# AndyWu0719/Audio-CALM

Measured on NVIDIA B200. Metric: log-mel audio-hours/sec, higher is better.
Workload: dtype f32

## Files before the change

### audio-calm_b200/csrc/acb_kernels.cu

```cuda
#include "audiocalm_b200.h"
#include "acb_fft32.cuh"

#include <cuda_bf16.h>
#include <cuda_runtime.h>

#include <algorithm>
#include <cmath>
#include <cstdio>
#include <cstring>
#include <mutex>
#include <numeric>
#include <string>
#include <vector>

namespace acb {

constexpr int kNfft = 1024;
constexpr int kHop = 256;
constexpr int kBins = 512;
constexpr int kTileFrames = 8;
constexpr int kGroupWarps = 4;
constexpr int kGroupThreads = kGroupWarps * 32;
constexpr int kMaxGroups = 4;
constexpr int kTileSamples = (kTileFrames + 3) * kHop;
constexpr int kRowStride = 36;
constexpr int kPlaneFloats = 32 * kRowStride;
constexpr int kScratchFloats = 2 * kPlaneFloats + 8;
constexpr int kSlots = 8;
constexpr int kMaxMels = 128;
constexpr int kMaxRounds = 4;
constexpr int kMaxWeights = 4096;
constexpr int kOutStageOffset = 2 * kBins;
static_assert(kScratchFloats % 32 == 8 && kScratchFloats % 4 == 0, "pair stride must be 8 (mod 32) words and 16-byte aligned");
static_assert(kOutStageOffset + kTileFrames * (kMaxMels | 1) <= kScratchFloats, "staged tile must fit above the power spectrum");

thread_local std::string g_last_error;

int fail(int code, const std::string& msg) {
    g_last_error = msg;
    return code;
}
static int cuda_fail(cudaError_t e, const char* what) {
    g_last_error = std::string(what) + ": " + cudaGetErrorString(e);
    return ACB_ERR_CUDA;
}
#define ACB_CUDA(call)                                  \
    do {                                                \
        cudaError_t e__ = (call);                       \
        if (e__ != cudaSuccess) return cuda_fail(e__, #call); \
    } while (0)

__device__ __forceinline__ unsigned smem_addr(const void* p) { return static_cast<unsigned>(__cvta_generic_to_shared(p)); }
__device__ __forceinline__ void mbar_init(unsigned long long* bar, unsigned count) {
    asm volatile("mbarrier.init.shared::cta.b64 [%0], %1;" ::"r"(smem_addr(bar)), "r"(count) : "memory");
}
__device__ __forceinline__ void mbar_arrive(unsigned long long* bar) {
    asm volatile("mbarrier.arrive.shared::cta.b64 _, [%0];" ::"r"(smem_addr(bar)) : "memory");
}
__device__ __forceinline__ void mbar_arrive_expect_tx(unsigned long long* bar, unsigned bytes) {
    asm volatile("mbarrier.arrive.expect_tx.shared::cta.b64 _, [%0], %1;" ::"r"(smem_addr(bar)), "r"(bytes) : "memory");
}
__device__ __forceinline__ bool mbar_wait(unsigned long long* bar, unsigned parity) {
    unsigned ok = 0;
    for (int spin = 0; spin < (1 << 26) && !ok; ++spin) {
        asm volatile("{\n\t.reg .pred p;\n\tmbarrier.try_wait.parity.shared::cta.b64 p, [%1], %2;\n\tselp.u32 %0, 1, 0, p;\n\t}\n"
                     : "=r"(ok) : "r"(smem_addr(bar)), "r"(parity) : "memory");
    }
    return ok != 0;
}
__device__ __forceinline__ void bulk_copy_g2s(void* smem, const void* gmem, unsigned bytes, unsigned long long* bar) {
    asm volatile("cp.async.bulk.shared::cluster.global.mbarrier::complete_tx::bytes [%0], [%1], %2, [%3];"
                 ::"r"(smem_addr(smem)), "l"(gmem), "r"(bytes), "r"(smem_addr(bar)) : "memory");
}

struct LogmelParams {
    const float* window;
    const float4* twiddle;
    const float* plan_w;
    const int* plan_woff;
    const short* plan_trip;
    const short* plan_band;
    const short* plan_astart;
    int n_plan_w;
    int n_mels;
    float clamp_min;
    float log_scale;
    float log_floor;
    const float* wav;
    const long long* clip_offset;
    const long long* clip_length;
    long long clip_stride;
    long long uniform_length;
    const int* tile_start;
    int n_clips;
    int n_tiles;
    int uniform_tiles_per_clip;
    const float* clip_peak;
    void* out;
    int out_bf16;
    int time_major;
    const long long* out_offset;
    long long out_clip_stride;
    long long frame_capacity;
    const long long* frame_capacity_per_clip;
    int pad_multiple;
    int fill_tail;
    float fill_value;
    int affine;
    float affine_mean;
    float affine_inv_std;
    const float* bin_mean;
    const float* bin_std;
    double* moments_partial;
    int* error_flag;
};

struct SmemLayout {
    int samples, scratch, twiddle, window, plan_w, affine, plan_rec, mbar, moments, total_bytes;
};

__host__ __device__ inline int out_row_stride(int n_mels) { return n_mels | 1; }

__host__ __device__ inline SmemLayout make_smem_layout(int kGroups, int n_mels, int n_plan_w, bool with_moments = false) {
    SmemLayout L;
    int off = 0;
    L.samples = off; off += kGroups * kTileSamples;
    L.scratch = off; off += kGroups * kGroupWarps * kScratchFloats;
    L.twiddle = off; off += 5 * 32 * 4;
    L.window = off; off += 32 * 20;
    if (!with_moments) {
        L.plan_rec = off; off += kGroupWarps * kMaxRounds * kSlots * 4;
        L.mbar = off; off += 2 * kGroups;
        off = (off + 3) & ~3;
        L.affine = off; off += 2 * kMaxMels;
        L.plan_w = off; off += (n_plan_w + 3) & ~3;
        L.moments = off;
    } else {
        L.plan_w = off; off += (n_plan_w + 3) & ~3;
        L.affine = off; off += 2 * ((n_mels + 1) & ~1);
        off = (off + 3) & ~3;
        L.plan_rec = off; off += kGroupWarps * kMaxRounds * kSlots * 4;
        L.mbar = off; off += 2 * kGroups;
        L.moments = off; off += kGroups * 4 * n_mels;
    }
    L.total_bytes = off * 4;
    return L;
}

struct ClipCursor {
    long long wav_base;
    long long length;
    long long out_base;
    int cap;
    int frames;
    int frames_padded;
    int clip;
    int tile_in_clip;
    int tiles_in_clip;
    float gain;
};

__device__ __forceinline__ void cursor_load_clip(const LogmelParams& p, ClipCursor& c) {
    const int i = c.clip;
    c.wav_base = p.clip_offset ? p.clip_offset[i] : (long long)i * p.clip_stride;
    c.length = p.clip_length ? p.clip_length[i] : p.uniform_length;
    c.out_base = p.out_offset ? p.out_offset[i] : (long long)i * p.out_clip_stride;
    c.cap = (int)(p.frame_capacity_per_clip ? p.frame_capacity_per_clip[i] : p.frame_capacity);
    c.frames = 1 + (int)(c.length / kHop);
    const int rem = c.frames % p.pad_multiple;
    c.frames_padded = rem ? c.frames + (p.pad_multiple - rem) : c.frames;
    c.tiles_in_clip = p.tile_start ? (__ldg(p.tile_start + i + 1) - __ldg(p.tile_start + i)) : p.uniform_tiles_per_clip;
    c.gain = 1.f;
    if (p.clip_peak) {
        const float peak = __ldg(p.clip_peak + i);
        if (peak > 0.f) {
            const float s = 0.95f / (peak + 1e-8f);
            c.gain = s * s;
        }
    }
}

__device__ __forceinline__ void cursor_init(const LogmelParams& p, ClipCursor& c, long long tile) {
    if (p.tile_start == nullptr) {
        c.clip = (int)(tile / p.uniform_tiles_per_clip);
        c.tile_in_clip = (int)(tile - (long long)c.clip * p.uniform_tiles_per_clip);
    } else {
        int lo = 0, hi = p.n_clips;
        while (hi - lo > 1) {
            const int mid = (lo + hi) >> 1;
            if ((long long)__ldg(p.tile_start + mid) <= tile) lo = mid; else hi = mid;
        }
        c.clip = lo;
        c.tile_in_clip = (int)(tile - __ldg(p.tile_start + lo));
    }
    cursor_load_clip(p, c);
}

__device__ __forceinline__ void cursor_advance(const LogmelParams& p, ClipCursor& c) {
    if (++c.tile_in_clip >= c.tiles_in_clip) {
        c.tile_in_clip = 0;
        do { ++c.clip; cursor_load_clip(p, c); } while (c.tiles_in_clip == 0 && c.clip + 1 < p.n_clips);
    }
}

__device__ __forceinline__ void group_sync(int grp) {
    asm volatile("bar.sync %0, %1;" ::"r"(grp + 1), "n"(kGroupThreads) : "memory");
}

__device__ __noinline__ void gather_edge_tile(const float* __restrict__ src, long long g0, long long L, float* s_samples, int gt) {
    static_assert(kTileSamples % kGroupThreads == 0, "whole rounds");
    float v[kTileSamples / kGroupThreads];
#pragma unroll
    for (int k = 0; k < kTileSamples / kGroupThreads; ++k) {
        long long idx = g0 + gt + k * kGroupThreads;
        if (idx < 0) idx = -idx;
        if (idx >= L) idx = 2 * (L - 1) - idx;
        v[k] = (idx >= 0 && idx < L) ? __ldg(src + idx) : 0.f;
    }
#pragma unroll
    for (int k = 0; k < kTileSamples / kGroupThreads; ++k) s_samples[gt + k * kGroupThreads] = v[k];
}

__device__ __forceinline__ void load_tile_samples(const LogmelParams& p, const ClipCursor& t, float* s_samples, int gt, int grp,
                                                  unsigned long long* full) {
    const int f0 = t.tile_in_clip * kTileFrames;
    const long long g0 = (long long)f0 * kHop - kNfft / 2;
    const float* src = p.wav + t.wav_base;
// ... 65 lines not shown
            v = p.fill_value;
        } else {
            continue;
        }
        const size_t e0 = p.time_major ? ((size_t)fr * n_mels + b) : ((size_t)b * c.cap + fr);
        out[e0] = to_out<OutT>(v);
        if (dup) {
            const int fd = 2 * T - 2 - fr;
            const size_t e1 = p.time_major ? ((size_t)fd * n_mels + b) : ((size_t)b * c.cap + fd);
            out[e1] = to_out<OutT>(v);
        }
    }
}

template <typename OutT>
__device__ __forceinline__ void fill_span(OutT* ptr, long long n, OutT fv, int t, int nt) {
    constexpr int per16 = 16 / (int)sizeof(OutT);
    const long long head = min(n, (long long)(((16 - (reinterpret_cast<uintptr_t>(ptr) & 15)) & 15) / sizeof(OutT)));
    for (long long i = t; i < head; i += nt) ptr[i] = fv;
    const long long body = (n - head) / per16;
    unsigned w;
    if (sizeof(OutT) == 4) w = *reinterpret_cast<const unsigned*>(&fv);
    else { const unsigned short h = *reinterpret_cast<const unsigned short*>(&fv); w = (unsigned)h | ((unsigned)h << 16); }
    uint4* q = reinterpret_cast<uint4*>(ptr + head);
    for (long long i = t; i < body; i += nt) q[i] = make_uint4(w, w, w, w);
    for (long long i = head + body * per16 + t; i < n; i += nt) ptr[i] = fv;
}

template <typename OutT>
__device__ __forceinline__ void fill_row_tail(const LogmelParams& p, const ClipCursor& c, int n_mels, int tid) {
    const int f_begin = (c.tile_in_clip + 1) * kTileFrames;
    const long long n_fill = (long long)c.cap - f_begin;
    if (n_fill <= 0) return;
    OutT* out = reinterpret_cast<OutT*>(p.out) + c.out_base;
    const OutT fv = to_out<OutT>(p.fill_value);
    if (p.time_major) {
        fill_span<OutT>(out + (size_t)f_begin * n_mels, n_fill * n_mels, fv, tid, kGroupThreads);
    } else {
        const int lane = tid & 31, warp = tid >> 5;
        for (int b = warp; b < n_mels; b += kGroupWarps) fill_span<OutT>(out + (size_t)b * c.cap + f_begin, n_fill, fv, lane, 32);
    }
}

__device__ __forceinline__ float lg2_normal(float x) {
    float y;
    asm("lg2.approx.ftz.f32 %0, %1;" : "=f"(y) : "f"(x));
    return y;
}

__device__ __forceinline__ void two_sum_add(float2& acc, float x) {
    const float t = __fadd_rn(acc.x, x);
    const float bb = __fsub_rn(t, acc.x);
    const float e = __fadd_rn(__fsub_rn(acc.x, __fsub_rn(t, bb)), __fsub_rn(x, bb));
    acc.y = __fadd_rn(acc.y, e);
    acc.x = t;
}

template <int G, bool kMoments, typename OutT>
__global__ void __launch_bounds__(G * kGroupThreads, G == 4 ? 1 : 2) logmel_fused_kernel(const LogmelParams p) {
    constexpr int kGroups = G;
    constexpr int kThreads = G * kGroupThreads;
    extern __shared__ __align__(16) float smem[];
    const SmemLayout L = make_smem_layout(G, p.n_mels, p.n_plan_w, kMoments);
    const int tid = threadIdx.x;
    const int lane = tid & 31;
    const int grp = tid / kGroupThreads;
    const int gt = tid % kGroupThreads;
    const int gw = gt >> 5;
    const int n_mels = p.n_mels;
    const int S = out_row_stride(n_mels);
    const bool write_out = p.out != nullptr;

    float* s_samples = smem + L.samples + grp * kTileSamples;
    float* s_scratch = smem + L.scratch + grp * kGroupWarps * kScratchFloats;
    float* s_out = s_scratch + kOutStageOffset;
    float4* s_tw4 = reinterpret_cast<float4*>(smem + L.twiddle);
    float* s_win = smem + L.window;
    float* s_pw = smem + L.plan_w;
    float2* s_aff = reinterpret_cast<float2*>(smem + L.affine);
    int4* s_rec = reinterpret_cast<int4*>(smem + L.plan_rec);
    float2* s_mom = reinterpret_cast<float2*>(smem + L.moments) + grp * 2 * n_mels;
    unsigned long long* s_full = reinterpret_cast<unsigned long long*>(smem + L.mbar) + grp;

    for (int i = tid; i < 5 * 32; i += kThreads) s_tw4[i] = p.twiddle[i];
    for (int i = tid; i < kNfft / 2; i += kThreads)
        s_win[(i & 31) * 20 + (i >> 5)] = p.window[i];
    for (int i = tid; i < p.n_plan_w; i += kThreads) s_pw[i] = p.plan_w[i];
    for (int i = tid; i < kGroupWarps * kMaxRounds * kSlots; i += kThreads) {
        const int slot = i / kSlots, qq = i - slot * kSlots;
        s_rec[i] = make_int4(p.plan_astart[i] >> 1, (p.plan_woff[slot] >> 1) + qq, p.plan_band[i], p.plan_trip[slot]);
    }
    for (int i = tid; i < n_mels; i += kThreads) {
        float sc = 1.f, sh = 0.f;
        if (p.affine == 1) { sc = p.affine_inv_std; sh = -p.affine_mean * p.affine_inv_std; }
        else if (p.affine == 2) { sc = 1.f / __ldg(p.bin_std + i); sh = -__ldg(p.bin_mean + i) * sc; }
        s_aff[i] = make_float2(sc, sh);
    }
    if (kMoments)
        for (int i = gt; i < 2 * n_mels; i += kGroupThreads) s_mom[i] = make_float2(0.f, 0.f);
    if (gt == 0) {
        mbar_init(s_full, 1);
        asm volatile("fence.mbarrier_init.release.cluster;" ::: "memory");
    }
    __syncthreads();

    const long long n_groups = (long long)gridDim.x * kGroups, g_index = (long long)blockIdx.x * kGroups + grp;
    const long long t_begin = (long long)p.n_tiles * g_index / n_groups;
    const long long t_end = (long long)p.n_tiles * (g_index + 1) / n_groups;

    ClipCursor cur;
    bool staged = false;
    unsigned full_parity = 0;
    if (t_begin < t_end) {
        cursor_init(p, cur, t_begin);
        staged = cur.tile_in_clip * kTileFrames < cur.frames;
        if (staged) load_tile_samples(p, cur, s_samples, gt, grp, s_full);
    }

    const int q = lane >> 2;
    const int pl = lane & 3;
    const float* pair_scratch = s_scratch + pl * kScratchFloats;
    float* scr = s_scratch + gw * kScratchFloats;
    float2* scr2 = reinterpret_cast<float2*>(scr);

    for (long long tile = t_begin; tile < t_end; ++tile) {
        if (staged) {
            if (!mbar_wait(s_full, full_parity) && lane == 0) atomicExch(p.error_flag, 1);
            full_parity ^= 1;
        }

        const int f0 = cur.tile_in_clip * kTileFrames;
        const bool has_frames = f0 < cur.frames;
        const bool active = has_frames && f0 + 2 * gw < cur.frames;

        if (active) {
            float2 pr[16], pi[16];
            {
                const float* sp = s_samples + (2 * gw) * kHop + lane;
                float2 v[20];
#pragma unroll
                for (int r = 0; r < 20; ++r) v[r] = make_float2(sp[32 * (2 * r)], sp[32 * (2 * r + 1)]);
                float4 w4[4];
                const float4* wq = reinterpret_cast<const float4*>(s_win + lane * 20);
#pragma unroll
                for (int u = 0; u < 4; ++u) w4[u] = wq[u];
#pragma unroll
                for (int j = 0; j < 8; ++j) {
                    const int t = brev5(2 * j) >> 1;
                    const float2 wa = (t & 1) ? make_float2(w4[t >> 1].z, w4[t >> 1].w) : make_float2(w4[t >> 1].x, w4[t >> 1].y);
                    const float2 br = __ffma2_rn(neg2(v[t + 8]), wa, v[t + 8]), bi = __ffma2_rn(neg2(v[t + 12]), wa, v[t + 12]);
                    pr[2 * j] = __ffma2_rn(v[t], wa, br);
                    pr[2 * j + 1] = __ffma2_rn(v[t], wa, neg2(br));
                    pi[2 * j] = __ffma2_rn(v[t + 4], wa, bi);
                    pi[2 * j + 1] = __ffma2_rn(v[t + 4], wa, neg2(bi));
                }
            }
            fft32_packed_from_stage2(pr, pi);
            group_sync(grp);
            {
                float* pre = scr + lane;
                float* pim = scr + kPlaneFloats + lane;
                float2 tr[4], ti[4];
#pragma unroll
                for (int c = 0; c < 4; ++c) {
                    const float4 sd = s_tw4[c * 32 + lane];
                    tr[c] = make_float2(sd.x, sd.y);
                    ti[c] = make_float2(sd.z, sd.w);
                }
                const float4 w4 = s_tw4[4 * 32 + lane];
                const float2 w4r = bcast2(w4.x), w4i = bcast2(w4.y);
#pragma unroll
                for (int k = 0; k < 16; ++k) {
                    const int c = k & 3;
                    const float2 yr = __ffma2_rn(neg2(pi[k]), ti[c], __fmul2_rn(pr[k], tr[c]));
                    const float2 yi = __ffma2_rn(pr[k], ti[c], __fmul2_rn(pi[k], tr[c]));
                    pre[k * kRowStride] = yr.x;
                    pre[(k + 16) * kRowStride] = yr.y;
                    pim[k * kRowStride] = yi.x;
                    pim[(k + 16) * kRowStride] = yi.y;
                    if (k + 4 < 16) {
                        const float2 nr = __ffma2_rn(neg2(ti[c]), w4i, __fmul2_rn(tr[c], w4r));
                        ti[c] = __ffma2_rn(tr[c], w4i, __fmul2_rn(ti[c], w4r));
                        tr[c] = nr;
                    }
                }
            }
            __syncwarp();
            {
                const float4* re4 = reinterpret_cast<const float4*>(scr + lane * kRowStride);
                const float4* im4 = reinterpret_cast<const float4*>(scr + kPlaneFloats + lane * kRowStride);
#pragma unroll
                for (int h = 0; h < 8; ++h) {
                    const float4 zr = re4[h], zi = im4[h];
                    pr[brev3(h)] = make_float2(zr.x, zr.y);
                    pr[brev3(h) + 8] = make_float2(zr.z, zr.w);
                    pi[brev3(h)] = make_float2(zi.x, zi.y);
                    pi[brev3(h) + 8] = make_float2(zi.z, zi.w);
                }
            }
// ... 454 lines not shown
                    T v[4];
#pragma unroll
                    for (int j = 0; j < 4; ++j) { const long long f = s0 + t + j; v[j] = (f >= 0 && f < n) ? src[f] : padv; }
                    *reinterpret_cast<float4*>(dst + t) = make_float4(v[0], v[1], v[2], v[3]);
                }
            }
        } else {
            for (long long t = lane; t < out_frames; t += 32) {
                const long long f = s0 + t;
                dst[t] = (f >= 0 && f < n) ? src[f] : padv;
            }
        }
    }
}

template <typename T>
__global__ void __launch_bounds__(256) pad_transpose_kernel(const T* __restrict__ feat, const long long* __restrict__ row_offset,
                                                            const long long* __restrict__ lens, int dim, T* __restrict__ out,
                                                            long long out_frames, float pad_value,
                                                            const long long* __restrict__ mask_start, const long long* __restrict__ mask_len) {
    constexpr int kT = 64;
    __shared__ float tile[kT][kT + 1];
    const int clip = blockIdx.z;
    const long long t0 = (long long)blockIdx.x * kT;
    const int d0 = blockIdx.y * kT;
    const long long n = lens[clip];
    const T* src = feat + row_offset[clip] * dim;
    const long long m0 = mask_start ? mask_start[clip] : 0, m1 = mask_start ? m0 + mask_len[clip] : 0;
    const int q = threadIdx.x & 15, r0 = threadIdx.x >> 4;
    const bool vec_in = sizeof(T) == 4 && (dim & 3) == 0 && (reinterpret_cast<uintptr_t>(src) & 15) == 0;
#pragma unroll
    for (int pass = 0; pass < kT / 16; ++pass) {
        const int r = pass * 16 + r0;
        const long long t = t0 + r;
        const int d = d0 + 4 * q;
        float v[4] = {pad_value, pad_value, pad_value, pad_value};
        if (t < n) {
            const bool masked = t >= m0 && t < m1;
            if (vec_in && d + 3 < dim) {
                if constexpr (sizeof(T) == 4) {
                    const float4 u = __ldg(reinterpret_cast<const float4*>(src + t * dim + d));
                    v[0] = u.x; v[1] = u.y; v[2] = u.z; v[3] = u.w;
                }
            } else {
#pragma unroll
                for (int j = 0; j < 4; ++j) if (d + j < dim) v[j] = (float)src[t * dim + d + j];
            }
            if (masked) { v[0] = v[1] = v[2] = v[3] = 0.f; }
        }
#pragma unroll
        for (int j = 0; j < 4; ++j) tile[4 * q + j][r] = v[j];
    }
    __syncthreads();
    const bool vec_out = sizeof(T) == 4 && (out_frames & 3) == 0 && (reinterpret_cast<uintptr_t>(out) & 15) == 0;
#pragma unroll
    for (int pass = 0; pass < kT / 16; ++pass) {
        const int r = pass * 16 + r0;
        const int d = d0 + r;
        const long long t = t0 + 4 * q;
        if (d >= dim || t >= out_frames) continue;
        T* dst = out + ((long long)clip * dim + d) * out_frames + t;
        if (vec_out && t + 3 < out_frames) {
            if constexpr (sizeof(T) == 4)
                *reinterpret_cast<float4*>(dst) = make_float4(tile[r][4 * q], tile[r][4 * q + 1], tile[r][4 * q + 2], tile[r][4 * q + 3]);
        } else {
#pragma unroll
            for (int j = 0; j < 4; ++j) if (t + j < out_frames) dst[j] = from_float<T>(tile[r][4 * q + j]);
        }
    }
}

}

struct acb_frontend {
    int device = 0;
    int n_fft = 0, hop = 0, n_mels = 0, n_weights = 0, log_kind = 0;
    float clamp_min = 0.f;
    int num_sms = 0;
    int groups = 0;
    int grid = 0;
    int smem_bytes = 0;
    int smem_bytes_moments = 0;
    void* d_blob = nullptr;
    const float* d_window = nullptr;
    const float4* d_twiddle = nullptr;
    const float* d_plan_w = nullptr;
    const int* d_plan_woff = nullptr;
    const short* d_plan_trip = nullptr;
    const short* d_plan_band = nullptr;
    const short* d_plan_astart = nullptr;
    int n_plan_w = 0;
    int* d_err = nullptr;
    cudaStream_t s_in = nullptr, s_out = nullptr;
    std::vector<cudaEvent_t> ev;
    std::mutex mu;
};

using namespace acb;

extern "C" {

int acb_abi_version(void) { return ACB_ABI_VERSION; }
const char* acb_last_error(void) { return g_last_error.c_str(); }
int acb_frames_per_tile(void) { return kTileFrames; }

int64_t acb_frames_for_length(int64_t length, int n_fft, int hop) {
    if (n_fft <= 0 || hop <= 0) return -1;
    if (length <= n_fft / 2) return -1;
    return 1 + length / hop;
}

int64_t acb_padded_frames(int64_t frames, int multiple) {
    if (multiple <= 1) return frames;
    const int64_t r = frames % multiple;
    return r ? frames + (multiple - r) : frames;
}

int64_t acb_plan_tiles(const int64_t* lengths_host, int32_t n_clips, int n_fft, int hop, int64_t frame_capacity,
                       int32_t* tile_start_host) {
    if (!lengths_host || !tile_start_host || n_clips < 0) return fail(ACB_ERR_INVALID, "acb_plan_tiles: null argument");
    int64_t total = 0;
    for (int32_t i = 0; i < n_clips; ++i) {
        const int64_t T = acb_frames_for_length(lengths_host[i], n_fft, hop);
        if (T < 0) {
            return fail(ACB_ERR_INVALID, "acb_plan_tiles: clip " + std::to_string(i) + " has " + std::to_string(lengths_host[i]) +
                                             " samples; reflect padding needs more than " + std::to_string(n_fft / 2));
        }
        const int64_t cover = frame_capacity > 0 ? frame_capacity : T;
        tile_start_host[i] = (int32_t)total;
        total += (cover + kTileFrames - 1) / kTileFrames;
        if (total > INT32_MAX) return fail(ACB_ERR_INVALID, "acb_plan_tiles: more than 2^31 tiles in one call");
    }
    tile_start_host[n_clips] = (int32_t)total;
    return total;
}

int acb_frontend_create(acb_frontend** out, int device, int n_fft, int hop, int n_mels, const float* window_host,
                        const float* fb_host, float clamp_min, int log_kind) {
    if (!out || !window_host || !fb_host) return fail(ACB_ERR_INVALID, "acb_frontend_create: null argument");
    if (n_fft != kNfft || hop != kHop)
        return fail(ACB_ERR_UNSUPPORTED, "acb_frontend_create: this build has kernels for n_fft=1024, hop=256 only (got n_fft=" +
                                             std::to_string(n_fft) + ", hop=" + std::to_string(hop) + ")");
    if (n_mels < 1 || n_mels > kMaxMels) return fail(ACB_ERR_UNSUPPORTED, "acb_frontend_create: n_mels must be in [1, 128]");
    if (log_kind != ACB_LOG_NATURAL && log_kind != ACB_LOG_10) return fail(ACB_ERR_INVALID, "acb_frontend_create: bad log_kind");
    if (!(clamp_min >= 1.17549435e-38f)) return fail(ACB_ERR_INVALID, "acb_frontend_create: clamp_min must be a positive normal float");
    for (int n = 0; n < kNfft / 2; ++n) {
        const double dev = std::fabs((double)window_host[n + kNfft / 2] - (1.0 - (double)window_host[n]));
        if (!(dev <= 1e-6))
            return fail(ACB_ERR_UNSUPPORTED, "acb_frontend_create: the window must have the periodic-Hann property w[n + 512] = 1 - w[n] "
                                             "(deviation " + std::to_string(dev) + " at n=" + std::to_string(n) + ")");
    }
    const int n_freq = n_fft / 2 + 1;

    std::vector<int> start(n_mels, 0), len(n_mels, 0), off(n_mels, 0);
    std::vector<float> weights;
    for (int m = 0; m < n_mels; ++m) {
        int lo = -1, hi = -1;
        for (int f = 0; f < n_freq; ++f)
            if (fb_host[(size_t)f * n_mels + m] != 0.f) { if (lo < 0) lo = f; hi = f; }
        off[m] = (int)weights.size();
        if (lo >= 0) {
            if (hi >= kBins) {
                if (fb_host[(size_t)(n_freq - 1) * n_mels + m] != 0.f)
                    return fail(ACB_ERR_UNSUPPORTED, "acb_frontend_create: filterbank has weight on the Nyquist bin");
            }
            start[m] = lo;
            len[m] = hi - lo + 1;
            for (int f = lo; f <= hi; ++f) weights.push_back(fb_host[(size_t)f * n_mels + m] * 0.25f);
        }
    }
    if ((int)weights.size() > kMaxWeights) return fail(ACB_ERR_UNSUPPORTED, "acb_frontend_create: filterbank too dense");

    std::vector<int> alen(n_mels), aend(n_mels);
// ... 2 lines not shown
        aend[m] = (start[m] + std::max(len[m], 1) + 1) & ~1;
        alen[m] = aend[m] - (start[m] & ~1);
    }
    std::vector<int> order(n_mels);
    std::iota(order.begin(), order.end(), 0);
    std::stable_sort(order.begin(), order.end(), [&](int a, int b) { return alen[a] > alen[b]; });
    const int n_rounds = (n_mels + kSlots - 1) / kSlots;
    std::vector<short> plan_band(kGroupWarps * kMaxRounds * kSlots, (short)-1), plan_astart(kGroupWarps * kMaxRounds * kSlots, (short)0),
        plan_trip(kGroupWarps * kMaxRounds, (short)0);
    std::vector<int> plan_woff(kGroupWarps * kMaxRounds, 0);
    std::vector<float> plan_w;
    std::vector<int> load(kGroupWarps, 0), rounds(kGroupWarps, 0);
    for (int g = 0; g < n_rounds; ++g) {
        int best = -1;
        for (int w = 0; w < kGroupWarps; ++w)
            if (rounds[w] < kMaxRounds && (best < 0 || load[w] < load[best])) best = w;
        if (best < 0) return fail(ACB_ERR_UNSUPPORTED, "acb_frontend_create: mel plan overflow");
        std::vector<int> par[2];
        for (int q = 0; q < kSlots && kSlots * g + q < n_mels; ++q) {
            const int m = order[kSlots * g + q];
            par[((start[m] & ~1) >> 1) & 1].push_back(m);
        }
        std::vector<int> slots;
        while (!par[0].empty() && !par[1].empty()) {
            slots.push_back(par[0].back()); par[0].pop_back();
            slots.push_back(par[1].back()); par[1].pop_back();
        }
        for (int k = 0; k < 2; ++k)
            for (int m : par[k]) slots.push_back(m);
        std::vector<int> shift(slots.size(), 0), as(slots.size(), 0);
        int trip = 2;
        for (int iter = 0; iter < 8; ++iter) {
            trip = 2;
            for (size_t i = 0; i < slots.size(); ++i) trip = std::max(trip, aend[slots[i]] - ((start[slots[i]] & ~1) - shift[i]));
            for (size_t i = 0; i < slots.size(); ++i) {
                as[i] = (start[slots[i]] & ~1) - shift[i];
                if (as[i] + trip > kBins) as[i] = std::max(0, (kBins - trip) & ~1);
            }
            bool changed = false;
            for (size_t i = 0; i + 1 < slots.size(); i += 2) {
                if ((((as[i] >> 1) ^ (as[i + 1] >> 1)) & 1) != 0) continue;
                const size_t x = (as[i + 1] >= 2 && (start[slots[i + 1]] & ~1) - shift[i + 1] == as[i + 1]) ? i + 1
                                 : ((as[i] >= 2 && (start[slots[i]] & ~1) - shift[i] == as[i]) ? i : slots.size());
                if (x < slots.size()) { shift[x] += 2; changed = true; }
            }
            if (!changed) break;
        }
        const int slot = best * kMaxRounds + rounds[best];
        plan_trip[slot] = (short)trip;
        plan_woff[slot] = (int)plan_w.size();
        plan_w.resize(plan_w.size() + (size_t)trip * kSlots, 0.f);
        float* wbase = plan_w.data() + plan_woff[slot];
        for (size_t q = 0; q < slots.size(); ++q) {
            const int m = slots[q];
            plan_band[slot * kSlots + q] = (short)m;
            plan_astart[slot * kSlots + q] = (short)as[q];
            for (int i = 0; i < len[m]; ++i) {
                const int rel = start[m] + i - as[q];
                if (rel < 0 || rel >= trip) return fail(ACB_ERR_UNSUPPORTED, "acb_frontend_create: mel plan window error");
                wbase[(rel >> 1) * (2 * kSlots) + q * 2 + (rel & 1)] = weights[off[m] + i];
            }
        }
        load[best] += trip + 16;
        rounds[best]++;
    }
    if ((int)plan_w.size() > kMaxWeights * 4) return fail(ACB_ERR_UNSUPPORTED, "acb_frontend_create: mel plan too large");

    std::vector<float4> tw(5 * 32);
    for (int l = 0; l < 32; ++l) {
        auto wre = [&](int m) { return (float)cos(-2.0 * M_PI * (double)(m * l) / 1024.0); };
        auto wim = [&](int m) { return (float)sin(-2.0 * M_PI * (double)(m * l) / 1024.0); };
        for (int k = 0; k < 4; ++k) tw[k * 32 + l] = make_float4(wre(k), wre(k + 16), wim(k), wim(k + 16));
        tw[4 * 32 + l] = make_float4(wre(4), wim(4), 0.f, 0.f);
    }

    int prev = 0;
    ACB_CUDA(cudaGetDevice(&prev));
    ACB_CUDA(cudaSetDevice(device));
    auto* fe = new acb_frontend();
    fe->device = device; fe->n_fft = n_fft; fe->hop = hop; fe->n_mels = n_mels; fe->n_weights = (int)weights.size();
    fe->n_plan_w = (int)plan_w.size();
    fe->log_kind = log_kind; fe->clamp_min = clamp_min;

    size_t o = 0;
    auto take = [&](size_t bytes) { size_t r = o; o += (bytes + 255) & ~size_t(255); return r; };
    const size_t o_win = take(sizeof(float) * kNfft), o_tw = take(sizeof(float4) * 160),
                 o_pw = take(sizeof(float) * std::max<size_t>(plan_w.size(), 1)), o_po = take(sizeof(int) * plan_woff.size()),
                 o_pt = take(sizeof(short) * plan_trip.size()), o_pb = take(sizeof(short) * plan_band.size()),
                 o_pa = take(sizeof(short) * plan_astart.size()), o_err = take(16);
    std::vector<unsigned char> host(o, 0);
    memcpy(host.data() + o_win, window_host, sizeof(float) * kNfft);
    memcpy(host.data() + o_tw, tw.data(), sizeof(float4) * 160);
    if (!plan_w.empty()) memcpy(host.data() + o_pw, plan_w.data(), sizeof(float) * plan_w.size());
    memcpy(host.data() + o_po, plan_woff.data(), sizeof(int) * plan_woff.size());
    memcpy(host.data() + o_pt, plan_trip.data(), sizeof(short) * plan_trip.size());
    memcpy(host.data() + o_pb, plan_band.data(), sizeof(short) * plan_band.size());
    memcpy(host.data() + o_pa, plan_astart.data(), sizeof(short) * plan_astart.size());
    cudaError_t e = cudaMalloc(&fe->d_blob, o);
    if (e == cudaSuccess) e = cudaMemcpy(fe->d_blob, host.data(), o, cudaMemcpyHostToDevice);
    cudaDeviceProp prop;
    if (e == cudaSuccess) e = cudaGetDeviceProperties(&prop, device);
    const int optin = (int)prop.sharedMemPerBlockOptin;
    fe->groups = std::max(make_smem_layout(kMaxGroups, n_mels, fe->n_plan_w, true).total_bytes,
                          make_smem_layout(kMaxGroups, n_mels, fe->n_plan_w, false).total_bytes) <= optin ? kMaxGroups : 2;
    const SmemLayout L = make_smem_layout(fe->groups, n_mels, fe->n_plan_w, false);
    const SmemLayout Lm = make_smem_layout(fe->groups, n_mels, fe->n_plan_w, true);
    fe->smem_bytes = L.total_bytes;
    fe->smem_bytes_moments = Lm.total_bytes;
    if (e == cudaSuccess && std::max(L.total_bytes, Lm.total_bytes) > optin) {
        if (fe->d_blob) cudaFree(fe->d_blob);
        delete fe;
        cudaSetDevice(prev);
        return fail(ACB_ERR_UNSUPPORTED, "acb_frontend_create: filterbank plan needs more shared memory than the device offers");
    }
    int occ = 0;
    auto prepare = [&](auto kernel, int threads) {
        if (e == cudaSuccess) e = cudaFuncSetAttribute(kernel, cudaFuncAttributeMaxDynamicSharedMemorySize, optin);
        if (e == cudaSuccess && occ == 0) e = cudaOccupancyMaxActiveBlocksPerMultiprocessor(&occ, kernel, threads, L.total_bytes);
    };
    if (fe->groups == 4) {
        prepare(logmel_fused_kernel<4, false, float>, 4 * kGroupThreads);
        prepare(logmel_fused_kernel<4, false, __nv_bfloat16>, 4 * kGroupThreads);
        prepare(logmel_fused_kernel<4, true, float>, 4 * kGroupThreads);
        prepare(logmel_fused_kernel<4, true, __nv_bfloat16>, 4 * kGroupThreads);
    } else {
        prepare(logmel_fused_kernel<2, false, float>, 2 * kGroupThreads);
        prepare(logmel_fused_kernel<2, false, __nv_bfloat16>, 2 * kGroupThreads);
        prepare(logmel_fused_kernel<2, true, float>, 2 * kGroupThreads);
        prepare(logmel_fused_kernel<2, true, __nv_bfloat16>, 2 * kGroupThreads);
    }
    if (e != cudaSuccess) {
        if (fe->d_blob) cudaFree(fe->d_blob);
        delete fe;
        cudaSetDevice(prev);
        return cuda_fail(e, "acb_frontend_create");
    }
    fe->num_sms = prop.multiProcessorCount;
    fe->grid = fe->num_sms * std::max(occ, 1);
    auto* base = static_cast<unsigned char*>(fe->d_blob);
    fe->d_window = reinterpret_cast<const float*>(base + o_win);
    fe->d_twiddle = reinterpret_cast<const float4*>(base + o_tw);
    fe->d_plan_w = reinterpret_cast<const float*>(base + o_pw);
    fe->d_plan_woff = reinterpret_cast<const int*>(base + o_po);
    fe->d_plan_trip = reinterpret_cast<const short*>(base + o_pt);
    fe->d_plan_band = reinterpret_cast<const short*>(base + o_pb);
    fe->d_plan_astart = reinterpret_cast<const short*>(base + o_pa);
    fe->d_err = reinterpret_cast<int*>(base + o_err);
    cudaSetDevice(prev);
    *out = fe;
    return ACB_OK;
}

int acb_frontend_destroy(acb_frontend* fe) {
    if (!fe) return ACB_OK;
    int prev = 0;
    cudaGetDevice(&prev);
    cudaSetDevice(fe->device);
    for (auto ev : fe->ev) cudaEventDestroy(ev);
    if (fe->s_in) cudaStreamDestroy(fe->s_in);
    if (fe->s_out) cudaStreamDestroy(fe->s_out);
    if (fe->d_blob) cudaFree(fe->d_blob);
    cudaSetDevice(prev);
    delete fe;
    return ACB_OK;
}

int64_t acb_moments_workspace_bytes(const acb_frontend* fe) {
    if (!fe) return fail(ACB_ERR_INVALID, "acb_moments_workspace_bytes: null handle");
    return (int64_t)fe->grid * fe->groups * 2 * fe->n_mels * (int64_t)sizeof(double);
}

int acb_logmel_forward(const acb_frontend* fe, const acb_logmel_args* a, void* stream) {
    if (!fe || !a) return fail(ACB_ERR_INVALID, "acb_logmel_forward: null argument");
    if (a->n_clips <= 0 || a->n_tiles <= 0) return ACB_OK;
    if (!a->wav) return fail(ACB_ERR_INVALID, "acb_logmel_forward: null wav");
    if (!a->out && !a->moments) return fail(ACB_ERR_INVALID, "acb_logmel_forward: out may be NULL only for a statistics-only launch (moments set)");
    if (a->out_dtype != ACB_F32 && a->out_dtype != ACB_BF16) return fail(ACB_ERR_INVALID, "acb_logmel_forward: bad out_dtype");
    if (a->out_layout != ACB_MEL_MAJOR && a->out_layout != ACB_TIME_MAJOR) return fail(ACB_ERR_INVALID, "acb_logmel_forward: bad out_layout");
    if (a->pad_multiple < 1) return fail(ACB_ERR_INVALID, "acb_logmel_forward: pad_multiple must be >= 1");
    if (kTileFrames % a->pad_multiple != 0)
        return fail(ACB_ERR_UNSUPPORTED, "acb_logmel_forward: pad_multiple must divide the " + std::to_string(kTileFrames) + "-frame tile (1, 2, 4 or 8)");
    if (a->affine < 0 || a->affine > 2) return fail(ACB_ERR_INVALID, "acb_logmel_forward: bad affine mode");
    if (a->affine == 2 && (!a->bin_mean || !a->bin_std)) return fail(ACB_ERR_INVALID, "acb_logmel_forward: per-bin affine needs bin_mean/bin_std");
    if (a->affine == 1 && !(a->affine_std > 0.f)) return fail(ACB_ERR_INVALID, "acb_logmel_forward: affine_std must be > 0");
    if (a->moments && !a->moments_workspace) return fail(ACB_ERR_INVALID, "acb_logmel_forward: moments need a workspace");
    if (!a->frame_capacity_per_clip && a->frame_capacity <= 0) return fail(ACB_ERR_INVALID, "acb_logmel_forward: frame_capacity must be > 0");
    if (a->frame_capacity * (int64_t)fe->n_mels >= (int64_t)1 << 32) return fail(ACB_ERR_INVALID, "acb_logmel_forward: n_mels * frame_capacity must be < 2^32");

    LogmelParams p{};
    p.window = fe->d_window; p.twiddle = fe->d_twiddle;
    p.plan_w = fe->d_plan_w; p.plan_woff = fe->d_plan_woff; p.plan_trip = fe->d_plan_trip;
    p.plan_band = fe->d_plan_band; p.plan_astart = fe->d_plan_astart; p.n_plan_w = fe->n_plan_w;
    p.n_mels = fe->n_mels; p.clamp_min = fe->clamp_min;
    p.log_scale = fe->log_kind == ACB_LOG_10 ? 0.30102999566398120f : 0.69314718055994531f;
    p.log_floor = fe->log_kind == ACB_LOG_10 ? log10f(fe->clamp_min) : logf(fe->clamp_min);
    p.wav = a->wav;
    p.clip_offset = reinterpret_cast<const long long*>(a->clip_offset);
    p.clip_length = reinterpret_cast<const long long*>(a->clip_length);
    p.clip_stride = a->clip_stride; p.uniform_length = a->uniform_length;
    p.tile_start = a->tile_start; p.n_clips = a->n_clips; p.n_tiles = a->n_tiles;
    p.uniform_tiles_per_clip = 1;
    if (!a->tile_start && a->clip_length) {
        if (!a->fill_tail || a->frame_capacity_per_clip)
            return fail(ACB_ERR_INVALID, "acb_logmel_forward: ragged clips need tile_start (acb_plan_tiles) unless fill_tail pads every clip to frame_capacity");
        p.uniform_tiles_per_clip = (int)((a->frame_capacity + kTileFrames - 1) / kTileFrames);
        if ((int64_t)p.uniform_tiles_per_clip * a->n_clips != a->n_tiles)
            return fail(ACB_ERR_INVALID, "acb_logmel_forward: n_tiles does not match n_clips * tiles per clip");
    } else if (!a->tile_start) {
        const int64_t T = acb_frames_for_length(a->uniform_length, fe->n_fft, fe->hop);
        if (T < 0) return fail(ACB_ERR_INVALID, "acb_logmel_forward: clips of " + std::to_string(a->uniform_length) +
                                                    " samples are too short for reflect padding of " + std::to_string(fe->n_fft / 2));
        const int64_t cover = a->fill_tail ? a->frame_capacity : T;
        p.uniform_tiles_per_clip = (int)((cover + kTileFrames - 1) / kTileFrames);
        if ((int64_t)p.uniform_tiles_per_clip * a->n_clips != a->n_tiles)
            return fail(ACB_ERR_INVALID, "acb_logmel_forward: n_tiles does not match n_clips * tiles per clip");
        if (acb_padded_frames(T, a->pad_multiple) > a->frame_capacity)
            return fail(ACB_ERR_INVALID, "acb_logmel_forward: frame_capacity smaller than the padded frame count");
        if (acb_padded_frames(T, a->pad_multiple) - T >= T)
            return fail(ACB_ERR_INVALID, "acb_logmel_forward: reflect pad to the multiple needs more frames than the clip has");
    }
    p.clip_peak = a->clip_peak;
    p.out = a->out; p.out_bf16 = a->out_dtype == ACB_BF16; p.time_major = a->out_layout == ACB_TIME_MAJOR;
    p.out_offset = reinterpret_cast<const long long*>(a->out_offset);
    p.out_clip_stride = a->out_clip_stride; p.frame_capacity = a->frame_capacity;
    p.frame_capacity_per_clip = reinterpret_cast<const long long*>(a->frame_capacity_per_clip);
    p.pad_multiple = a->pad_multiple; p.fill_tail = a->fill_tail; p.fill_value = a->fill_value;
    p.affine = a->affine; p.affine_mean = a->affine_mean;
    p.affine_inv_std = a->affine == 1 ? (float)(1.0 / (double)a->affine_std) : 1.f;
    p.bin_mean = a->bin_mean; p.bin_std = a->bin_std;
    p.moments_partial = a->moments ? static_cast<double*>(a->moments_workspace) : nullptr;
    p.error_flag = fe->d_err;

    int prev = 0;
    ACB_CUDA(cudaGetDevice(&prev));
    if (prev != fe->device) ACB_CUDA(cudaSetDevice(fe->device));
    cudaStream_t st = static_cast<cudaStream_t>(stream);
    const int grid = fe->grid;
    const int threads = fe->groups * kGroupThreads;
    const size_t smem = a->moments ? fe->smem_bytes_moments : fe->smem_bytes;
    auto launch = [&](auto kernel) { kernel<<<grid, threads, smem, st>>>(p); };
    if (fe->groups == 4) {
        if (a->moments) { if (p.out_bf16) launch(logmel_fused_kernel<4, true, __nv_bfloat16>); else launch(logmel_fused_kernel<4, true, float>); }
        else { if (p.out_bf16) launch(logmel_fused_kernel<4, false, __nv_bfloat16>); else launch(logmel_fused_kernel<4, false, float>); }
    } else {
        if (a->moments) { if (p.out_bf16) launch(logmel_fused_kernel<2, true, __nv_bfloat16>); else launch(logmel_fused_kernel<2, true, float>); }
        else { if (p.out_bf16) launch(logmel_fused_kernel<2, false, __nv_bfloat16>); else launch(logmel_fused_kernel<2, false, float>); }
    }
    if (a->moments) {
        const int n_vals = 2 * fe->n_mels;
        moments_reduce_kernel<<<(n_vals + 7) / 8, 256, 0, st>>>(p.moments_partial, grid * fe->groups, n_vals, a->moments);
    }
    cudaError_t e = cudaGetLastError();
    if (prev != fe->device) cudaSetDevice(prev);
    if (e != cudaSuccess) return cuda_fail(e, "acb_logmel_forward launch");
    return ACB_OK;
}

int acb_frontend_set_kernel(acb_frontend* fe, int kind) {
    if (!fe) return fail(ACB_ERR_INVALID, "acb_frontend_set_kernel: null handle");
    if (kind < 0 || kind > 2) return fail(ACB_ERR_INVALID, "acb_frontend_set_kernel: kind must be 0 (automatic), 1 (CUDA-core mel) or 2 (tensor-core mel)");
    if (kind == 2) return fail(ACB_ERR_UNSUPPORTED, "acb_frontend_set_kernel: this build has only the CUDA-core mel kernel (kind 0 or 1)");
    return ACB_OK;
}

int acb_frontend_check(const acb_frontend* fe, void* stream) {
    if (!fe) return fail(ACB_ERR_INVALID, "acb_frontend_check: null handle");
    int flag = 0, prev = 0;
    ACB_CUDA(cudaGetDevice(&prev));
    if (prev != fe->device) ACB_CUDA(cudaSetDevice(fe->device));
    cudaError_t e = cudaStreamSynchronize(static_cast<cudaStream_t>(stream));
    if (e == cudaSuccess) e = cudaMemcpy(&flag, fe->d_err, sizeof(int), cudaMemcpyDeviceToHost);
    if (e == cudaSuccess && flag) cudaMemset(fe->d_err, 0, sizeof(int));
    if (prev != fe->device) cudaSetDevice(prev);
    if (e != cudaSuccess) return cuda_fail(e, "acb_frontend_check");
    if (flag) return fail(ACB_ERR_CUDA, "acb_frontend_check: a sample-tile copy did not complete inside the kernel (results are invalid)");
// ... 275 lines not shown
```

Baseline: 4554.

## Pack constant tables into one image and bulk-copy it with TMA at block start

Precomputes the twiddle, window, plan records and filterbank weights on the host into a single contiguous image in the final shared-memory layout. In the main kernel one thread issues cp.async.bulk copies tracked by an mbarrier, overlapping them with the first tile's sample load and the affine setup, instead of having every thread gather and transform the tables from separate global arrays. The aim is to shorten per-block prologue latency. It adds dependence on layout matching between host image and smem offsets, plus another barrier.

After: 4593 (median of 6 runs). No clear change (+0.9%).

```diff
diff --git a/audio-calm_b200/csrc/acb_kernels.cu b/audio-calm_b200/csrc/acb_kernels.cu
--- a/audio-calm_b200/csrc/acb_kernels.cu
+++ b/audio-calm_b200/csrc/acb_kernels.cu
@@ -60,6 +60,9 @@
 __device__ __forceinline__ void mbar_arrive_expect_tx(unsigned long long* bar, unsigned bytes) {
     asm volatile("mbarrier.arrive.expect_tx.shared::cta.b64 _, [%0], %1;" ::"r"(smem_addr(bar)), "r"(bytes) : "memory");
 }
+__device__ __forceinline__ void mbar_expect_tx(unsigned long long* bar, unsigned bytes) {
+    asm volatile("mbarrier.expect_tx.shared::cta.b64 [%0], %1;" ::"r"(smem_addr(bar)), "r"(bytes) : "memory");
+}
 __device__ __forceinline__ bool mbar_wait(unsigned long long* bar, unsigned parity) {
     unsigned ok = 0;
     for (int spin = 0; spin < (1 << 26) && !ok; ++spin) {
@@ -74,13 +77,7 @@
 }
 
 struct LogmelParams {
-    const float* window;
-    const float4* twiddle;
-    const float* plan_w;
-    const int* plan_woff;
-    const short* plan_trip;
-    const short* plan_band;
-    const short* plan_astart;
+    const float* tables;
     int n_plan_w;
     int n_mels;
     float clamp_min;
@@ -116,7 +113,14 @@
 };
 
 struct SmemLayout {
-    int samples, scratch, twiddle, window, plan_w, affine, plan_rec, mbar, moments, total_bytes;
+    int samples, scratch, twiddle, window, plan_w, affine, plan_rec, mbar, moments, tables_bar, total_bytes;
+};
+
+struct TableImage {
+    static constexpr int kTwWin = 5 * 32 * 4 + 32 * 20;
+    static constexpr int kRec = kGroupWarps * kMaxRounds * kSlots * 4;
+    __host__ __device__ static int plan_w_words(int n_plan_w) { return (n_plan_w + 3) & ~3; }
+    __host__ __device__ static int words(int n_plan_w) { return kTwWin + kRec + plan_w_words(n_plan_w); }
 };
 
 __host__ __device__ inline int out_row_stride(int n_mels) { return n_mels | 1; }
@@ -143,6 +147,7 @@
         L.mbar = off; off += 2 * kGroups;
         L.moments = off; off += kGroups * 4 * n_mels;
     }
+    L.tables_bar = off; off += 2;
     L.total_bytes = off * 4;
     return L;
 }
@@ -374,27 +379,39 @@
     float2* s_mom = reinterpret_cast<float2*>(smem + L.moments) + grp * 2 * n_mels;
     unsigned long long* s_full = reinterpret_cast<unsigned long long*>(smem + L.mbar) + grp;
 
-    for (int i = tid; i < 5 * 32; i += kThreads) s_tw4[i] = p.twiddle[i];
-    for (int i = tid; i < kNfft / 2; i += kThreads)
-        s_win[(i & 31) * 20 + (i >> 5)] = p.window[i];
-    for (int i = tid; i < p.n_plan_w; i += kThreads) s_pw[i] = p.plan_w[i];
-    for (int i = tid; i < kGroupWarps * kMaxRounds * kSlots; i += kThreads) {
-        const int slot = i / kSlots, qq = i - slot * kSlots;
-        s_rec[i] = make_int4(p.plan_astart[i] >> 1, (p.plan_woff[slot] >> 1) + qq, p.plan_band[i], p.plan_trip[slot]);
-    }
-    for (int i = tid; i < n_mels; i += kThreads) {
-        float sc = 1.f, sh = 0.f;
-        if (p.affine == 1) { sc = p.affine_inv_std; sh = -p.affine_mean * p.affine_inv_std; }
-        else if (p.affine == 2) { sc = 1.f / __ldg(p.bin_std + i); sh = -__ldg(p.bin_mean + i) * sc; }
-        s_aff[i] = make_float2(sc, sh);
-    }
-    if (kMoments)
+    unsigned long long* s_tables = reinterpret_cast<unsigned long long*>(smem + L.tables_bar);
+    if (kMoments) {
+        const float4* img = reinterpret_cast<const float4*>(p.tables);
+        float4* s_img = reinterpret_cast<float4*>(s_tw4);
+        for (int i = tid; i < TableImage::kTwWin / 4; i += kThreads) s_img[i] = img[i];
+        for (int i = tid; i < TableImage::kRec / 4; i += kThreads) s_rec[i] = reinterpret_cast<const int4*>(img + TableImage::kTwWin / 4)[i];
+        for (int i = tid; i < TableImage::plan_w_words(p.n_plan_w) / 4; i += kThreads)
+            reinterpret_cast<float4*>(s_pw)[i] = img[(TableImage::kTwWin + TableImage::kRec) / 4 + i];
+        for (int i = tid; i < n_mels; i += kThreads) {
+            float sc = 1.f, sh = 0.f;
+            if (p.affine == 1) { sc = p.affine_inv_std; sh = -p.affine_mean * p.affine_inv_std; }
+            else if (p.affine == 2) { sc = 1.f / __ldg(p.bin_std + i); sh = -__ldg(p.bin_mean + i) * sc; }
+            s_aff[i] = make_float2(sc, sh);
+        }
         for (int i = gt; i < 2 * n_mels; i += kGroupThreads) s_mom[i] = make_float2(0.f, 0.f);
-    if (gt == 0) {
-        mbar_init(s_full, 1);
+        if (gt == 0) {
+            mbar_init(s_full, 1);
+            asm volatile("fence.mbarrier_init.release.cluster;" ::: "memory");
+        }
+        __syncthreads();
+    } else if (tid == 0) {
+        for (int g = 0; g < kGroups; ++g) mbar_init(reinterpret_cast<unsigned long long*>(smem + L.mbar) + g, 1);
+        mbar_init(s_tables, kThreads);
         asm volatile("fence.mbarrier_init.release.cluster;" ::: "memory");
     }
-    __syncthreads();
+    if (!kMoments) __syncthreads();
+    if (!kMoments && tid == 0) {
+        const int pw_words = TableImage::plan_w_words(p.n_plan_w);
+        mbar_expect_tx(s_tables, TableImage::words(p.n_plan_w) * 4u);
+        bulk_copy_g2s(s_tw4, p.tables, TableImage::kTwWin * 4u, s_tables);
+        bulk_copy_g2s(s_rec, p.tables + TableImage::kTwWin, TableImage::kRec * 4u, s_tables);
+        bulk_copy_g2s(s_pw, p.tables + TableImage::kTwWin + TableImage::kRec, pw_words * 4u, s_tables);
+    }
 
     const long long n_groups = (long long)gridDim.x * kGroups, g_index = (long long)blockIdx.x * kGroups + grp;
     const long long t_begin = (long long)p.n_tiles * g_index / n_groups;
@@ -407,6 +424,17 @@
         cursor_init(p, cur, t_begin);
         staged = cur.tile_in_clip * kTileFrames < cur.frames;
         if (staged) load_tile_samples(p, cur, s_samples, gt, grp, s_full);
+    }
+
+    if (!kMoments) {
+        for (int i = tid; i < n_mels; i += kThreads) {
+            float sc = 1.f, sh = 0.f;
+            if (p.affine == 1) { sc = p.affine_inv_std; sh = -p.affine_mean * p.affine_inv_std; }
+            else if (p.affine == 2) { sc = 1.f / __ldg(p.bin_std + i); sh = -__ldg(p.bin_mean + i) * sc; }
+            s_aff[i] = make_float2(sc, sh);
+        }
+        mbar_arrive(s_tables);
+        if (!mbar_wait(s_tables, 0) && lane == 0) atomicExch(p.error_flag, 1);
     }
 
     const int q = lane >> 2;
@@ -1027,13 +1055,7 @@
     int smem_bytes = 0;
     int smem_bytes_moments = 0;
     void* d_blob = nullptr;
-    const float* d_window = nullptr;
-    const float4* d_twiddle = nullptr;
-    const float* d_plan_w = nullptr;
-    const int* d_plan_woff = nullptr;
-    const short* d_plan_trip = nullptr;
-    const short* d_plan_band = nullptr;
-    const short* d_plan_astart = nullptr;
+    const float* d_tables = nullptr;
     int n_plan_w = 0;
     int* d_err = nullptr;
     cudaStream_t s_in = nullptr, s_out = nullptr;
@@ -1202,20 +1224,18 @@
     fe->n_plan_w = (int)plan_w.size();
     fe->log_kind = log_kind; fe->clamp_min = clamp_min;
 
-    size_t o = 0;
-    auto take = [&](size_t bytes) { size_t r = o; o += (bytes + 255) & ~size_t(255); return r; };
-    const size_t o_win = take(sizeof(float) * kNfft), o_tw = take(sizeof(float4) * 160),
-                 o_pw = take(sizeof(float) * std::max<size_t>(plan_w.size(), 1)), o_po = take(sizeof(int) * plan_woff.size()),
-                 o_pt = take(sizeof(short) * plan_trip.size()), o_pb = take(sizeof(short) * plan_band.size()),
-                 o_pa = take(sizeof(short) * plan_astart.size()), o_err = take(16);
+    std::vector<float> image(TableImage::words(fe->n_plan_w), 0.f);
+    memcpy(image.data(), tw.data(), sizeof(float4) * 160);
+    for (int i = 0; i < kNfft / 2; ++i) image[5 * 32 * 4 + (i & 31) * 20 + (i >> 5)] = window_host[i];
+    int4* rec = reinterpret_cast<int4*>(image.data() + TableImage::kTwWin);
+    for (int i = 0; i < kGroupWarps * kMaxRounds * kSlots; ++i) {
+        const int slot = i / kSlots, q = i - slot * kSlots;
+        rec[i] = make_int4(plan_astart[i] >> 1, (plan_woff[slot] >> 1) + q, plan_band[i], plan_trip[slot]);
+    }
+    std::copy(plan_w.begin(), plan_w.end(), image.begin() + TableImage::kTwWin + TableImage::kRec);
+    const size_t o_err = (image.size() * sizeof(float) + 255) & ~size_t(255), o = o_err + 16;
     std::vector<unsigned char> host(o, 0);
-    memcpy(host.data() + o_win, window_host, sizeof(float) * kNfft);
-    memcpy(host.data() + o_tw, tw.data(), sizeof(float4) * 160);
-    if (!plan_w.empty()) memcpy(host.data() + o_pw, plan_w.data(), sizeof(float) * plan_w.size());
-    memcpy(host.data() + o_po, plan_woff.data(), sizeof(int) * plan_woff.size());
-    memcpy(host.data() + o_pt, plan_trip.data(), sizeof(short) * plan_trip.size());
-    memcpy(host.data() + o_pb, plan_band.data(), sizeof(short) * plan_band.size());
-    memcpy(host.data() + o_pa, plan_astart.data(), sizeof(short) * plan_astart.size());
+    memcpy(host.data(), image.data(), image.size() * sizeof(float));
     cudaError_t e = cudaMalloc(&fe->d_blob, o);
     if (e == cudaSuccess) e = cudaMemcpy(fe->d_blob, host.data(), o, cudaMemcpyHostToDevice);
     cudaDeviceProp prop;
@@ -1258,13 +1278,7 @@
     fe->num_sms = prop.multiProcessorCount;
     fe->grid = fe->num_sms * std::max(occ, 1);
     auto* base = static_cast<unsigned char*>(fe->d_blob);
-    fe->d_window = reinterpret_cast<const float*>(base + o_win);
-    fe->d_twiddle = reinterpret_cast<const float4*>(base + o_tw);
-    fe->d_plan_w = reinterpret_cast<const float*>(base + o_pw);
-    fe->d_plan_woff = reinterpret_cast<const int*>(base + o_po);
-    fe->d_plan_trip = reinterpret_cast<const short*>(base + o_pt);
-    fe->d_plan_band = reinterpret_cast<const short*>(base + o_pb);
-    fe->d_plan_astart = reinterpret_cast<const short*>(base + o_pa);
+    fe->d_tables = reinterpret_cast<const float*>(base);
     fe->d_err = reinterpret_cast<int*>(base + o_err);
     cudaSetDevice(prev);
     *out = fe;
@@ -1308,9 +1322,7 @@
     if (a->frame_capacity * (int64_t)fe->n_mels >= (int64_t)1 << 32) return fail(ACB_ERR_INVALID, "acb_logmel_forward: n_mels * frame_capacity must be < 2^32");
 
     LogmelParams p{};
-    p.window = fe->d_window; p.twiddle = fe->d_twiddle;
-    p.plan_w = fe->d_plan_w; p.plan_woff = fe->d_plan_woff; p.plan_trip = fe->d_plan_trip;
-    p.plan_band = fe->d_plan_band; p.plan_astart = fe->d_plan_astart; p.n_plan_w = fe->n_plan_w;
+    p.tables = fe->d_tables; p.n_plan_w = fe->n_plan_w;
     p.n_mels = fe->n_mels; p.clamp_min = fe->clamp_min;
     p.log_scale = fe->log_kind == ACB_LOG_10 ? 0.30102999566398120f : 0.69314718055994531f;
     p.log_floor = fe->log_kind == ACB_LOG_10 ? log10f(fe->clamp_min) : logf(fe->clamp_min);
```
